# Edward-Sun/DIFUSCO

Hardware: NVIDIA H100
Metric: TSP-500 graphs/sec, 50-step categorical denoise (higher is better)
Workload: dtype f32 (3-term bf16 split on wgmma, fp32 accumulate)

## Files before the change

difusco_b200/csrc/edge_layer_tc.cuh:

```cuda
#pragma once
#include <cuda.h>
#include <cuda_bf16.h>
#include <cuda_runtime.h>

#include <stdlib.h>

#include <string>

#include "common.cuh"
#include "edge_layer_fp32.cuh"

namespace dfb {

constexpr int WG_ROWS = 64;
constexpr int TC_KBLK = 64;
constexpr int TC_KCH = 32;
constexpr int TC_B_BYTES = 256 * TC_KCH * 2;
static_assert(TC_KCH * 2 == 64, "weight chunk rows are one 64-byte swizzle row (tensor map, wgmma_desc_sw64)");
constexpr int TC_A_CHUNK = WG_ROWS * 128;
constexpr int TC_A_BYTES = 8 * TC_A_CHUNK;
constexpr int CONV_BATCH = 16;

constexpr int W_LO_ROWS = H;
constexpr int W_MAT_ROWS = 2 * W_LO_ROWS;
constexpr int W_LAYER_ROWS = 6 * W_MAT_ROWS;
__host__ __device__ constexpr int w_row_C(int l) { return l * W_LAYER_ROWS; }
__host__ __device__ constexpr int w_row_O(int l) { return w_row_C(l) + W_MAT_ROWS; }
__host__ __device__ constexpr int w_row_UVAB(int l) { return w_row_C(l) + 2 * W_MAT_ROWS; }
__host__ __device__ constexpr int w_row_embed(int L, int which) { return L * W_LAYER_ROWS + which * W_MAT_ROWS; }
__host__ __device__ constexpr int w_arena_rows(int L) { return w_row_embed(L, 2); }

template <int NWG>
struct TcCfg {
  static_assert(NWG == 1 || NWG == 2, "one or two consumer warpgroups");
  static constexpr int TILE = NWG * WG_ROWS;
  static constexpr int THREADS = (NWG + 1) * 128;
  static constexpr int NSTAGE = 2 * TC_KBLK / TC_KCH;
  static constexpr int OFF_B = NWG * TC_A_BYTES;
  static constexpr int OFF_PRM = OFF_B + NSTAGE * TC_B_BYTES;
  static constexpr int OFF_ROW = OFF_PRM + 6 * H * 4;
  static constexpr int OFF_SRC = OFF_ROW + TILE * 4;
  static constexpr int OFF_BAR = OFF_SRC + TILE * 8;
  static constexpr int SMEM_BYTES = OFF_BAR + 2 * NSTAGE * 8;
  static constexpr int SMEM_ALLOC = SMEM_BYTES + 1024;
  static constexpr int OFF_TAU = SMEM_BYTES;
  static constexpr int SMEM_ALLOC_TROWS = SMEM_ALLOC + TILE * 8;
  static_assert(SMEM_ALLOC_TROWS <= 232448, "shared memory budget (227 KB per block)");
};

struct TcParams {
  float* e;
  const float* uvab;
  float* partials;
  GraphDev g;
  LayerParams lp;
  const float* tvec;
  const float* xt_lut;
  const float* lut;
  const float* zero_row;
  float* debug_acc;
  const float* lin_in;
  float* lin_out;
  const float* lin_bias;
  int lin_rows;
  int lin_nb;
  int lin_w_row;
  int* error_flag;
  unsigned long long* phase_cycles;
  int write_e, e_zero, agg_mode;
  int w_row_base;
  int n_tiles;
  TimeRows trows;
};

__device__ __forceinline__ uint32_t smem_u32(const void* p) { return (uint32_t)__cvta_generic_to_shared(p); }

__device__ __forceinline__ void mbar_init(uint64_t* bar, uint32_t count) {
  asm volatile("mbarrier.init.shared::cta.b64 [%0], %1;" ::"r"(smem_u32(bar)), "r"(count) : "memory");
}
__device__ __forceinline__ void mbar_arrive(uint64_t* bar) {
  asm volatile("mbarrier.arrive.shared::cta.b64 _, [%0];" ::"r"(smem_u32(bar)) : "memory");
}
__device__ __forceinline__ void mbar_arrive_expect_tx(uint64_t* bar, uint32_t bytes) {
  asm volatile("mbarrier.arrive.expect_tx.shared::cta.b64 _, [%0], %1;" ::"r"(smem_u32(bar)), "r"(bytes) : "memory");
}
__device__ __forceinline__ void mbar_wait(uint64_t* bar, uint32_t parity, int* error_flag, int code) {
  const uint32_t addr = smem_u32(bar);
  uint32_t ok = 0;
#pragma unroll 1
  for (uint32_t spin = 0;; ++spin) {
    asm volatile(
        "{\n .reg .pred p;\n mbarrier.try_wait.parity.shared::cta.b64 p, [%1], %2, %3;\n selp.u32 %0, 1, 0, p;\n}"
        : "=r"(ok)
        : "r"(addr), "r"(parity), "r"(20000u)
        : "memory");
    if (ok) return;
    if (spin > 400000u) {
      if (error_flag) {
        error_flag[1] = (int)blockIdx.x;
        error_flag[2] = (int)parity;
        error_flag[3] = (int)threadIdx.x;
        atomicExch(error_flag, code);
      }
      __threadfence_system();
      __trap();
    }
  }
}
__device__ __forceinline__ void tma_load_2d(uint32_t dst, const CUtensorMap* map, uint64_t* bar, int c0, int c1) {
  asm volatile(
      "cp.async.bulk.tensor.2d.shared::cluster.global.mbarrier::complete_tx::bytes [%0], [%1, {%3, %4}], [%2];"
      ::"r"(dst), "l"(reinterpret_cast<uint64_t>(map)), "r"(smem_u32(bar)), "r"(c0), "r"(c1)
      : "memory");
}
__device__ __forceinline__ void fence_proxy_async() { asm volatile("fence.proxy.async.shared::cta;" ::: "memory"); }
__device__ __forceinline__ void cp_async16(void* dst, const void* src) {
  asm volatile("cp.async.cg.shared.global [%0], [%1], 16;" ::"r"(smem_u32(dst)), "l"(src) : "memory");
}
__device__ __forceinline__ void cp_async_commit() { asm volatile("cp.async.commit_group;" ::: "memory"); }
__device__ __forceinline__ void cp_async_wait_all() { asm volatile("cp.async.wait_group 0;" ::: "memory"); }

__device__ __forceinline__ uint64_t wgmma_desc_sw128(uint32_t smem_addr) {
  return (uint64_t)((smem_addr >> 4) & 0x3fffu) | (1ull << 16) | (64ull << 32) | (1ull << 62);
}
__device__ __forceinline__ uint64_t wgmma_desc_sw64(uint32_t smem_addr) {
  return (uint64_t)((smem_addr >> 4) & 0x3fffu) | (1ull << 16) | (32ull << 32) | (2ull << 62);
}
__device__ __forceinline__ void wgmma_fence() { asm volatile("wgmma.fence.sync.aligned;" ::: "memory"); }
__device__ __forceinline__ void wgmma_commit() { asm volatile("wgmma.commit_group.sync.aligned;" ::: "memory"); }
template <int N>
__device__ __forceinline__ void wgmma_wait() { asm volatile("wgmma.wait_group.sync.aligned %0;" ::"n"(N) : "memory"); }
__device__ __forceinline__ void acc_fence(float (&d)[128]) {
#pragma unroll
  for (int i = 0; i < 128; ++i) asm volatile("" : "+f"(d[i])::"memory");
}
__device__ __forceinline__ void wgmma_bf16(float (&d)[128], uint64_t da, uint64_t db, uint32_t scale_d) {
  asm volatile(
      "{\n .reg .pred p;\n setp.ne.b32 p, %130, 0;\n"
      "wgmma.mma_async.sync.aligned.m64n256k16.f32.bf16.bf16 "
      "{%0, %1, %2, %3, %4, %5, %6, %7, %8, %9, %10, %11, %12, %13, %14, %15, "
      "%16, %17, %18, %19, %20, %21, %22, %23, %24, %25, %26, %27, %28, %29, %30, %31, "
      "%32, %33, %34, %35, %36, %37, %38, %39, %40, %41, %42, %43, %44, %45, %46, %47, "
      "%48, %49, %50, %51, %52, %53, %54, %55, %56, %57, %58, %59, %60, %61, %62, %63, "
      "%64, %65, %66, %67, %68, %69, %70, %71, %72, %73, %74, %75, %76, %77, %78, %79, "
      "%80, %81, %82, %83, %84, %85, %86, %87, %88, %89, %90, %91, %92, %93, %94, %95, "
      "%96, %97, %98, %99, %100, %101, %102, %103, %104, %105, %106, %107, %108, %109, %110, %111, "
      "%112, %113, %114, %115, %116, %117, %118, %119, %120, %121, %122, %123, %124, %125, %126, %127}, "
      "%128, %129, p, 1, 1, 0, 0;\n}"
      : "+f"(d[0]), "+f"(d[1]), "+f"(d[2]), "+f"(d[3]), "+f"(d[4]), "+f"(d[5]), "+f"(d[6]), "+f"(d[7]),
        "+f"(d[8]), "+f"(d[9]), "+f"(d[10]), "+f"(d[11]), "+f"(d[12]), "+f"(d[13]), "+f"(d[14]), "+f"(d[15]),
        "+f"(d[16]), "+f"(d[17]), "+f"(d[18]), "+f"(d[19]), "+f"(d[20]), "+f"(d[21]), "+f"(d[22]), "+f"(d[23]),
        "+f"(d[24]), "+f"(d[25]), "+f"(d[26]), "+f"(d[27]), "+f"(d[28]), "+f"(d[29]), "+f"(d[30]), "+f"(d[31]),
        "+f"(d[32]), "+f"(d[33]), "+f"(d[34]), "+f"(d[35]), "+f"(d[36]), "+f"(d[37]), "+f"(d[38]), "+f"(d[39]),
        "+f"(d[40]), "+f"(d[41]), "+f"(d[42]), "+f"(d[43]), "+f"(d[44]), "+f"(d[45]), "+f"(d[46]), "+f"(d[47]),
        "+f"(d[48]), "+f"(d[49]), "+f"(d[50]), "+f"(d[51]), "+f"(d[52]), "+f"(d[53]), "+f"(d[54]), "+f"(d[55]),
        "+f"(d[56]), "+f"(d[57]), "+f"(d[58]), "+f"(d[59]), "+f"(d[60]), "+f"(d[61]), "+f"(d[62]), "+f"(d[63]),
        "+f"(d[64]), "+f"(d[65]), "+f"(d[66]), "+f"(d[67]), "+f"(d[68]), "+f"(d[69]), "+f"(d[70]), "+f"(d[71]),
        "+f"(d[72]), "+f"(d[73]), "+f"(d[74]), "+f"(d[75]), "+f"(d[76]), "+f"(d[77]), "+f"(d[78]), "+f"(d[79]),
        "+f"(d[80]), "+f"(d[81]), "+f"(d[82]), "+f"(d[83]), "+f"(d[84]), "+f"(d[85]), "+f"(d[86]), "+f"(d[87]),
        "+f"(d[88]), "+f"(d[89]), "+f"(d[90]), "+f"(d[91]), "+f"(d[92]), "+f"(d[93]), "+f"(d[94]), "+f"(d[95]),
        "+f"(d[96]), "+f"(d[97]), "+f"(d[98]), "+f"(d[99]), "+f"(d[100]), "+f"(d[101]), "+f"(d[102]), "+f"(d[103]),
        "+f"(d[104]), "+f"(d[105]), "+f"(d[106]), "+f"(d[107]), "+f"(d[108]), "+f"(d[109]), "+f"(d[110]), "+f"(d[111]),
        "+f"(d[112]), "+f"(d[113]), "+f"(d[114]), "+f"(d[115]), "+f"(d[116]), "+f"(d[117]), "+f"(d[118]), "+f"(d[119]),
        "+f"(d[120]), "+f"(d[121]), "+f"(d[122]), "+f"(d[123]), "+f"(d[124]), "+f"(d[125]), "+f"(d[126]), "+f"(d[127])
      : "l"(da), "l"(db), "r"(scale_d));
}

__device__ __forceinline__ float sigmoid_mufu(float x) {
  float t, r;
  asm("ex2.approx.ftz.f32 %0, %1;" : "=f"(t) : "f"(-1.4426950408889634f * x));
  asm("rcp.approx.ftz.f32 %0, %1;" : "=f"(r) : "f"(1.0f + t));
  return r;
}
__device__ __forceinline__ void split4(float4 x, uint2& hi, uint2& lo) {
  __nv_bfloat162 h01 = __floats2bfloat162_rn(x.x, x.y), h23 = __floats2bfloat162_rn(x.z, x.w);
  float2 f01 = __bfloat1622float2(h01), f23 = __bfloat1622float2(h23);
  __nv_bfloat162 l01 = __floats2bfloat162_rn(x.x - f01.x, x.y - f01.y);
  __nv_bfloat162 l23 = __floats2bfloat162_rn(x.z - f23.x, x.w - f23.y);
  hi.x = *reinterpret_cast<uint32_t*>(&h01);
  hi.y = *reinterpret_cast<uint32_t*>(&h23);
  lo.x = *reinterpret_cast<uint32_t*>(&l01);
  lo.y = *reinterpret_cast<uint32_t*>(&l23);
}
__device__ __forceinline__ void split2(float a, float b, uint32_t& hi, uint32_t& lo) {
  __nv_bfloat162 h = __floats2bfloat162_rn(a, b);
  const float2 f = __bfloat1622float2(h);
  __nv_bfloat162 l = __floats2bfloat162_rn(a - f.x, b - f.y);
  hi = *reinterpret_cast<uint32_t*>(&h);
  lo = *reinterpret_cast<uint32_t*>(&l);
}
__device__ __forceinline__ uint32_t sw128_off(int r, int j) {
  return (uint32_t)((r >> 3) * 1024 + (r & 7) * 128 + ((j ^ (r & 7)) << 4));
}
__device__ __forceinline__ int msg_col(int j, int r) { return 64 * (j >> 3) + ((8 * (j & 7)) ^ (8 * (r & 7))); }
__device__ __forceinline__ float quad_sum(float v) {
  v += __shfl_xor_sync(0xffffffffu, v, 1);
  return v + __shfl_xor_sync(0xffffffffu, v, 2);
}
__device__ __forceinline__ void swap_row_halves(float (&d)[128]) {
#pragma unroll
  for (int j = 0; j < 32; ++j) {
    const float x0 = d[4 * j], x1 = d[4 * j + 1];
    d[4 * j] = d[4 * j + 2];
    d[4 * j + 1] = d[4 * j + 3];
    d[4 * j + 2] = x0;
    d[4 * j + 3] = x1;
  }
}

enum {
  PH_TILES = 0,
  PH_TOTAL,
  PH_CONVERT,
  PH_G1_WAIT,
  PH_G1_MMA,
  PH_E1,
  PH_REDUCE,
  PH_LN,
  PH_G2_WAIT,
  PH_G2_MMA,
  PH_E4,
  PH_COUNT
};

template <int NWG, bool LIN, bool TIMED = false, bool TROWS = false>
__device__ __forceinline__ void edge_layer_wg_body(const CUtensorMap& wmap, const TcParams& P) {
  using Cfg = TcCfg<NWG>;
  constexpr int NSTAGE = Cfg::NSTAGE;
  extern __shared__ unsigned char smem_raw[];
  unsigned char* smem = smem_raw + ((1024u - (smem_u32(smem_raw) & 1023u)) & 1023u);
  float* prm = reinterpret_cast<float*>(smem + Cfg::OFF_PRM);
  int* s_row = reinterpret_cast<int*>(smem + Cfg::OFF_ROW);
  const float** s_src = reinterpret_cast<const float**>(smem + Cfg::OFF_SRC);
  const float** s_tau = reinterpret_cast<const float**>(smem + Cfg::OFF_TAU);
  uint64_t* full = reinterpret_cast<uint64_t*>(smem + Cfg::OFF_BAR);
  uint64_t* empty = full + NSTAGE;

  const int warp = threadIdx.x >> 5, lane = threadIdx.x & 31;
  constexpr bool lin = LIN;
  const int loads_per_tile = (P.write_e ? 2 : 1) * NWG * 4 * NSTAGE;

  if (threadIdx.x == 0) {
    for (int s = 0; s < NSTAGE; ++s) {
      mbar_init(&full[s], 1);
      mbar_init(&empty[s], 4);
    }
    asm volatile("fence.mbarrier_init.release.cluster;" ::: "memory");
    fence_proxy_async();
  }
  for (int i = threadIdx.x; i < H; i += Cfg::THREADS) {
    prm[i] = P.lp.ln_e_g[i];
    prm[H + i] = P.lp.ln_e_b[i];
    prm[2 * H + i] = P.tvec ? P.tvec[i] : 0.0f;
    prm[3 * H + i] = P.lp.ln_o_g[i];
    prm[4 * H + i] = P.lp.ln_o_b[i];
    prm[5 * H + i] = P.lp.b_O[i];
  }
  __syncthreads();
  const uint32_t smem_base = smem_u32(smem);

  if (warp >= 4 * NWG) {
    if constexpr (NWG == 2) asm volatile("setmaxnreg.dec.sync.aligned.u32 40;" ::: "memory");
    if (warp == 4 * NWG && lane == 0) {
      uint32_t u = 0;
      for (int tile = blockIdx.x; tile < P.n_tiles; tile += gridDim.x) {
        for (int i = 0; i < loads_per_tile; ++i, ++u) {
          const int s = u % NSTAGE;
          mbar_wait(&empty[s], ((u / NSTAGE) & 1) ^ 1, P.error_flag, 1);
          mbar_arrive_expect_tx(&full[s], TC_B_BYTES);
          const int row = (lin ? P.lin_w_row + (P.lin_nb == 4 ? (tile & 3) : 0) * W_MAT_ROWS
                               : P.w_row_base + (i >= 4 * NSTAGE * NWG ? w_row_O(0) - w_row_C(0) : 0)) +
                          (s >= NSTAGE / 2 ? W_LO_ROWS : 0);
          const int k = ((i / NSTAGE) & 3) * TC_KBLK + (s % (NSTAGE / 2)) * TC_KCH;
          tma_load_2d(smem_base + Cfg::OFF_B + s * TC_B_BYTES, &wmap, &full[s], k, row);
        }
      }
    }
    return;
  }

  if constexpr (NWG == 2) asm volatile("setmaxnreg.inc.sync.aligned.u32 232;" ::: "memory");
  const int wg = warp >> 2, wi = warp & 3, tid = threadIdx.x & 127;
  const int t4 = lane & 3;
  const int lr0 = wi * 16 + (lane >> 2);
  unsigned char* a_reg = smem + wg * TC_A_BYTES;
  const uint32_t a_base = smem_base + wg * TC_A_BYTES;
  float* msg = reinterpret_cast<float*>(a_reg);
  int* w_row = s_row + wg * WG_ROWS;
  const float** w_src = s_src + wg * WG_ROWS;
  const float** w_tau = s_tau + wg * WG_ROWS;
  auto wg_bar = [&] { asm volatile("bar.sync %0, 128;" ::"r"(1 + wg) : "memory"); };
  const int n_rows = lin ? P.lin_rows : P.g.E;
  float acc[128];

  auto turn_wait = [&] {
    if constexpr (NWG == 2) asm volatile("bar.sync %0, 256;" ::"r"(3 + wg) : "memory");
  };
  auto turn_pass = [&] {
    if constexpr (NWG == 2) asm volatile("bar.arrive %0, 256;" ::"r"(4 - wg) : "memory");
  };
  if (wg == 1) turn_pass();

  uint32_t t_mark = 0, t_start = 0;
  if constexpr (TIMED) t_start = t_mark = (uint32_t)clock();
  auto record = [&](int slot, uint32_t v) {
    if constexpr (TIMED) {
      if (tid == 0) atomicAdd(P.phase_cycles + slot, (unsigned long long)v);
    }
  };
  auto mark = [&](int slot) {
    if constexpr (TIMED) {
      const uint32_t now = (uint32_t)clock();
      record(slot, now - t_mark);
      t_mark = now;
    }
  };

  auto gemm = [&](int wait_slot, int mma_slot) {
    uint32_t waited = 0;
    turn_wait();
    if constexpr (TIMED) t_mark = (uint32_t)clock();
    acc_fence(acc);
    wgmma_fence();
#pragma unroll 1
    for (int kc = 0; kc < 4; ++kc) {
      const uint32_t ahi = a_base + kc * 2 * TC_A_CHUNK, alo = ahi + TC_A_CHUNK;
#pragma unroll
      for (int s = 0; s < NSTAGE; ++s) {
        uint32_t w0 = 0;
        if constexpr (TIMED) w0 = (uint32_t)clock();
        mbar_wait(&full[s], kc & 1, P.error_flag, 2);
        if constexpr (TIMED) waited += (uint32_t)clock() - w0;
        const uint32_t b = smem_base + Cfg::OFF_B + s * TC_B_BYTES;
        const bool b_hi = s < NSTAGE / 2;
#pragma unroll
        for (int k = 0; k < TC_KCH / 16; ++k) {
          const int ks = (s % (NSTAGE / 2)) * (TC_KCH / 16) + k;
          const uint64_t db = wgmma_desc_sw64(b + k * 32);
          wgmma_bf16(acc, wgmma_desc_sw128(ahi + ks * 32), db, (b_hi && ks == 0) ? (uint32_t)(kc != 0) : 1u);
          if (b_hi) wgmma_bf16(acc, wgmma_desc_sw128(alo + ks * 32), db, 1u);
        }
        wgmma_commit();
        wgmma_wait<1>();
        __syncwarp();
        if (lane == 0 && (s > 0 || kc > 0)) mbar_arrive(&empty[(s + NSTAGE - 1) % NSTAGE]);
      }
    }
    wgmma_wait<0>();
    acc_fence(acc);
    __syncwarp();
    if (lane == 0) mbar_arrive(&empty[NSTAGE - 1]);
    turn_pass();
    if constexpr (TIMED) {
      const uint32_t now = (uint32_t)clock();
      record(wait_slot, waited);
      record(mma_slot, now - t_mark - waited);
      t_mark = now;
    }
  };

  auto stage_rows = [&](auto row_src) {
#pragma unroll 1
    for (int i = 0; i < 16; ++i) {
      const int r = wi * 16 + i;
      const float* src = row_src(i) + 4 * lane;
      float* dst = msg + r * H + ((4 * lane) ^ (8 * (r & 7)));
      cp_async16(dst, src);
      cp_async16(dst + 128, src + 128);
    }
    cp_async_commit();
  };

  for (int tile = blockIdx.x; tile < P.n_tiles; tile += gridDim.x) {
    record(PH_TILES, 1);
    const int row_tile = (lin && P.lin_nb == 4) ? (tile >> 2) : tile;
    const int s_base = row_tile * Cfg::TILE + wg * WG_ROWS;
    if (tid < WG_ROWS) {
      const int s = s_base + tid;
      const float* src = P.zero_row;
      int rw = -1;
      if (s < n_rows && lin) {
        src = P.lin_in + (size_t)s * H;
      } else if (s < n_rows) {
        rw = P.g.row[s];
        if (P.e_zero) src = P.zero_row;
        else if (P.xt_lut) src = P.lut + ((P.xt_lut[P.g.perm ? P.g.perm[s] : s] != 0.0f) ? H : 0);
        else src = P.e + (size_t)s * H;
      }
      w_row[tid] = rw;
      w_src[tid] = src;
      if constexpr (TROWS) w_tau[tid] = s < n_rows ? time_row(P.tvec, P.trows, P.g.perm ? P.g.perm[s] : s) : P.zero_row;
    }
    wg_bar();

#pragma unroll 1
    for (int it0 = 0; it0 < 32; it0 += CONV_BATCH) {
      float4 x[CONV_BATCH];
#pragma unroll
      for (int q = 0; q < CONV_BATCH; ++q) {
        const int item = (it0 + q) * 128 + tid;
        x[q] = __ldcg(reinterpret_cast<const float4*>(w_src[item >> 6]) + (item & 63));
      }
#pragma unroll
      for (int q = 0; q < CONV_BATCH; ++q) {
        const int item = (it0 + q) * 128 + tid;
        const int rr = item >> 6, k4 = item & 63;
        uint2 hi, lo;
        split4(x[q], hi, lo);
        const uint32_t off = (k4 >> 4) * 2 * TC_A_CHUNK + sw128_off(rr, (k4 & 15) >> 1) + (k4 & 1) * 8;
        *reinterpret_cast<uint2*>(a_reg + off) = hi;
        *reinterpret_cast<uint2*>(a_reg + off + TC_A_CHUNK) = lo;
      }
    }
    fence_proxy_async();
    wg_bar();
    mark(PH_CONVERT);
    gemm(PH_G1_WAIT, PH_G1_MMA);

    const int sa = s_base + lr0, sb = sa + 8;
    const bool va = sa < n_rows, vb = sb < n_rows;
    if (lin || P.debug_acc) {
      const int nb = (lin && P.lin_nb == 4) ? (tile & 3) : 0;
      const int ostride = lin ? P.lin_nb * H : H;
      float* out = lin ? P.lin_out + nb * H : P.debug_acc;
#pragma unroll
      for (int h = 0; h < 2; ++h) {
        const int s = h ? sb : sa;
        if (!(h ? vb : va)) continue;
#pragma unroll
        for (int j = 0; j < 32; ++j) {
          const int c = 8 * j + 2 * t4;
          float2 o = make_float2(acc[4 * j + 2 * h], acc[4 * j + 2 * h + 1]);
          if (lin) {
            const float2 bb = __ldg(reinterpret_cast<const float2*>(P.lin_bias + nb * H + c));
            o.x += bb.x;
            o.y += bb.y;
          }
          __stcg(reinterpret_cast<float2*>(out + (size_t)s * ostride + c), o);
        }
      }
      continue;
    }

    const int s_lane = s_base + wi * 16 + (lane & 15);
    const int col_lane = s_lane < n_rows ? P.g.col[s_lane] : 0;
    stage_rows([&](int i) { return P.uvab + (size_t)__shfl_sync(0xffffffffu, col_lane, i) * 4 * H + H; });
#pragma unroll 1
    for (int h = 0; h < 2; ++h) {
      const bool v = h ? vb : va;
      const float* ap = P.uvab + (size_t)__shfl_sync(0xffffffffu, col_lane, (lane >> 2) + 8 * h) * 4 * H + 2 * H;
      const float* bp = P.uvab + (size_t)(v ? P.g.row[h ? sb : sa] : 0) * 4 * H + 3 * H;
#pragma unroll
      for (int j = 0; j < 32; ++j) {
        const int c = 8 * j + 2 * t4;
        const float2 ah = __ldg(reinterpret_cast<const float2*>(ap + c));
        const float2 bh = __ldg(reinterpret_cast<const float2*>(bp + c));
        acc[4 * j] = (acc[4 * j] + ah.x) + bh.x;
        acc[4 * j + 1] = (acc[4 * j + 1] + ah.y) + bh.y;
      }
      if (h == 0) {
        cp_async_wait_all();
        __syncwarp();
      }
      float* m = msg + (lr0 + 8 * h) * H + 2 * t4;
#pragma unroll
      for (int j = 0; j < 32; ++j) {
        float2* mp = reinterpret_cast<float2*>(m + msg_col(j, lr0));
        const float2 vh = *mp;
        *mp = make_float2(sigmoid_mufu(acc[4 * j]) * vh.x, sigmoid_mufu(acc[4 * j + 1]) * vh.y);
      }
      swap_row_halves(acc);
    }
    wg_bar();
    mark(PH_E1);
    const bool amax = P.agg_mode == AGG_MAX;
    const float run0 = amax ? -INFINITY : 0.0f;
#pragma unroll 1
    for (int g2 = 0; g2 < WG_ROWS / GROUP; ++g2) {
      const int grp = (s_base >> 5) + g2;
      if (grp >= P.g.n_groups) break;
      const int first_node = P.g.grp_first[grp];
      const size_t pair_base = (size_t)P.g.grp_pair[grp];
      const int node = w_row[g2 * GROUP + lane];
      const int nxt = __shfl_down_sync(0xffffffffu, node, 1);
      const uint32_t ends = __ballot_sync(0xffffffffu, node >= 0 && (lane == GROUP - 1 || nxt != node));
#pragma unroll 1
      for (int cc = 0; cc < 2; ++cc) {
        const int c = tid + 128 * cc;
        float run = run0;
#pragma unroll 8
        for (int r = 0; r < GROUP; ++r) {
          const int lr = g2 * GROUP + r;
          const float m = msg[lr * H + (c ^ (8 * (lr & 7)))];
          run = amax ? fmaxf(run, m) : run + m;
          if ((ends >> r) & 1u) {
            P.partials[(pair_base + (size_t)(w_row[lr] - first_node)) * H + c] = run;
            run = run0;
          }
        }
      }
    }
    wg_bar();
    mark(PH_REDUCE);
    if (!P.write_e) continue;

#pragma unroll 1
    for (int h = 0; h < 2; ++h) {
      float sum = 0.f;
#pragma unroll
      for (int j = 0; j < 32; ++j) sum += acc[4 * j] + acc[4 * j + 1];
      float mean = quad_sum(sum) * (1.0f / H);
      float q = 0.f;
#pragma unroll
      for (int j = 0; j < 32; ++j) {
        const float d0 = acc[4 * j] - mean, d1 = acc[4 * j + 1] - mean;
        q = fmaf(d0, d0, fmaf(d1, d1, q));
      }
      float rstd = rsqrtf(quad_sum(q) * (1.0f / H) + LN_EPS);
      sum = 0.f;
      const float* tau = nullptr;
      if constexpr (TROWS) tau = w_tau[lr0 + 8 * h];
#pragma unroll
      for (int j = 0; j < 32; ++j) {
        const int c = 8 * j + 2 * t4;
        const float2 g = *reinterpret_cast<const float2*>(prm + c);
        const float2 b = *reinterpret_cast<const float2*>(prm + H + c);
        float2 t;
        if constexpr (TROWS) t = __ldg(reinterpret_cast<const float2*>(tau + c));
        else t = *reinterpret_cast<const float2*>(prm + 2 * H + c);
        const float y0 = fmaxf(fmaf((acc[4 * j] - mean) * rstd, g.x, b.x), 0.0f) + t.x;
        const float y1 = fmaxf(fmaf((acc[4 * j + 1] - mean) * rstd, g.y, b.y), 0.0f) + t.y;
        acc[4 * j] = y0;
        acc[4 * j + 1] = y1;
        sum += y0 + y1;
      }
      mean = quad_sum(sum) * (1.0f / H);
      q = 0.f;
#pragma unroll
      for (int j = 0; j < 32; ++j) {
        const float d0 = acc[4 * j] - mean, d1 = acc[4 * j + 1] - mean;
        q = fmaf(d0, d0, fmaf(d1, d1, q));
      }
      rstd = rsqrtf(quad_sum(q) * (1.0f / H) + LN_EPS);
      const int r = lr0 + 8 * h;
#pragma unroll
      for (int j = 0; j < 32; ++j) {
        const int c = 8 * j + 2 * t4;
        const float2 g = *reinterpret_cast<const float2*>(prm + 3 * H + c);
        const float2 b = *reinterpret_cast<const float2*>(prm + 4 * H + c);
        const float z0 = fmaf((acc[4 * j] - mean) * rstd, g.x, b.x);
        const float z1 = fmaf((acc[4 * j + 1] - mean) * rstd, g.y, b.y);
        uint32_t hi, lo;
        split2(z0 * sigmoid_mufu(z0), z1 * sigmoid_mufu(z1), hi, lo);
        const uint32_t off = (j >> 3) * 2 * TC_A_CHUNK + sw128_off(r, j & 7) + 4 * t4;
        *reinterpret_cast<uint32_t*>(a_reg + off) = hi;
        *reinterpret_cast<uint32_t*>(a_reg + off + TC_A_CHUNK) = lo;
      }
      swap_row_halves(acc);
    }
    const float* e_src = w_src[wi * 16 + (lane & 15)];
    fence_proxy_async();
    wg_bar();
    mark(PH_LN);
    gemm(PH_G2_WAIT, PH_G2_MMA);

    stage_rows([&](int i) {
      return reinterpret_cast<const float*>(__shfl_sync(0xffffffffu, reinterpret_cast<unsigned long long>(e_src), i));
    });
    cp_async_wait_all();
    __syncwarp();
#pragma unroll
    for (int h = 0; h < 2; ++h) {
      if (!(h ? vb : va)) continue;
      const int r = lr0 + 8 * h;
      const float* er = msg + r * H + 2 * t4;
      float* dst = P.e + (size_t)(h ? sb : sa) * H;
#pragma unroll
      for (int j = 0; j < 32; ++j) {
        const int c = 8 * j + 2 * t4;
        const float2 ein = *reinterpret_cast<const float2*>(er + msg_col(j, r));
        const float2 bo = *reinterpret_cast<const float2*>(prm + 5 * H + c);
        __stcg(reinterpret_cast<float2*>(dst + c),
               make_float2((ein.x + acc[4 * j + 2 * h]) + bo.x, (ein.y + acc[4 * j + 2 * h + 1]) + bo.y));
      }
    }
    mark(PH_E4);
  }
  if constexpr (TIMED) record(PH_TOTAL, (uint32_t)clock() - t_start);
}

__global__ void __launch_bounds__(TcCfg<2>::THREADS, 1)
k_edge_layer_wg2(const __grid_constant__ CUtensorMap wmap, const TcParams P) {
  edge_layer_wg_body<2, false>(wmap, P);
}
__global__ void __launch_bounds__(TcCfg<2>::THREADS, 1)
k_edge_layer_wg2_timed(const __grid_constant__ CUtensorMap wmap, const TcParams P) {
  edge_layer_wg_body<2, false, true>(wmap, P);
}
__global__ void __launch_bounds__(TcCfg<1>::THREADS, 1)
k_edge_layer_wg1(const __grid_constant__ CUtensorMap wmap, const TcParams P) {
  edge_layer_wg_body<1, false>(wmap, P);
}
__global__ void __launch_bounds__(TcCfg<2>::THREADS, 1)
k_edge_layer_wg2_trows(const __grid_constant__ CUtensorMap wmap, const TcParams P) {
  edge_layer_wg_body<2, false, false, true>(wmap, P);
}
__global__ void __launch_bounds__(TcCfg<1>::THREADS, 1)
k_edge_layer_wg1_trows(const __grid_constant__ CUtensorMap wmap, const TcParams P) {
  edge_layer_wg_body<1, false, false, true>(wmap, P);
}
__global__ void __launch_bounds__(TcCfg<2>::THREADS, 1)
k_linear_wg2(const __grid_constant__ CUtensorMap wmap, const TcParams P) {
  edge_layer_wg_body<2, true>(wmap, P);
}

struct TcState {
  std::string err;
  int num_sms = 0;
  CUtensorMap wmap;
  bool bound = false;
  float* zero_row = nullptr;
  int* error_flag = nullptr;
  int* error_host = nullptr;
  unsigned long long* phase_cycles = nullptr;

  TcState() = default;
  TcState(const TcState&) = delete;
  TcState& operator=(const TcState&) = delete;
  ~TcState() {
    if (zero_row) cudaFree(zero_row);
    if (error_host) cudaFreeHost(error_host);
    if (phase_cycles) cudaFree(phase_cycles);
  }
};

typedef CUresult (*PFN_encodeTiled)(CUtensorMap*, CUtensorMapDataType, cuuint32_t, void*, const cuuint64_t*,
                                    const cuuint64_t*, const cuuint32_t*, const cuuint32_t*, CUtensorMapInterleave,
                                    CUtensorMapSwizzle, CUtensorMapL2promotion, CUtensorMapFloatOOBfill);

inline int tc_init(TcState* st, int num_sms) {
  st->num_sms = num_sms;
  cudaError_t e = cudaFuncSetAttribute(k_edge_layer_wg2, cudaFuncAttributeMaxDynamicSharedMemorySize, TcCfg<2>::SMEM_ALLOC);
  if (e == cudaSuccess)
    e = cudaFuncSetAttribute(k_edge_layer_wg2_timed, cudaFuncAttributeMaxDynamicSharedMemorySize, TcCfg<2>::SMEM_ALLOC);
  if (e == cudaSuccess)
    e = cudaFuncSetAttribute(k_edge_layer_wg1, cudaFuncAttributeMaxDynamicSharedMemorySize, TcCfg<1>::SMEM_ALLOC);
  if (e == cudaSuccess)
    e = cudaFuncSetAttribute(k_edge_layer_wg2_trows, cudaFuncAttributeMaxDynamicSharedMemorySize, TcCfg<2>::SMEM_ALLOC_TROWS);
  if (e == cudaSuccess)
    e = cudaFuncSetAttribute(k_edge_layer_wg1_trows, cudaFuncAttributeMaxDynamicSharedMemorySize, TcCfg<1>::SMEM_ALLOC_TROWS);
  if (e == cudaSuccess)
    e = cudaFuncSetAttribute(k_linear_wg2, cudaFuncAttributeMaxDynamicSharedMemorySize, TcCfg<2>::SMEM_ALLOC);
  if (e != cudaSuccess) {
    st->err = std::string("cudaFuncSetAttribute: ") + cudaGetErrorString(e);
    return -2;
  }
  if ((e = cudaMalloc(&st->zero_row, H * sizeof(float))) != cudaSuccess ||
      (e = cudaMemset(st->zero_row, 0, H * sizeof(float))) != cudaSuccess ||
      (e = cudaMalloc(&st->phase_cycles, 32 * sizeof(unsigned long long))) != cudaSuccess ||
      (e = cudaMemset(st->phase_cycles, 0, 32 * sizeof(unsigned long long))) != cudaSuccess ||
      (e = cudaHostAlloc(&st->error_host, 4 * sizeof(int), cudaHostAllocMapped)) != cudaSuccess ||
      (e = cudaHostGetDevicePointer((void**)&st->error_flag, st->error_host, 0)) != cudaSuccess) {
    st->err = std::string("tc_init alloc: ") + cudaGetErrorString(e);
    return -2;
  }
  return 0;
}

inline int tc_bind_weights(TcState* st, const uint16_t* arena, int L) {
  void* fn = nullptr;
  cudaDriverEntryPointQueryResult qres;
  cudaError_t e = cudaGetDriverEntryPoint("cuTensorMapEncodeTiled", &fn, cudaEnableDefault, &qres);
  if (e != cudaSuccess || !fn || qres != cudaDriverEntryPointSuccess) {
    st->err = "cuTensorMapEncodeTiled entry point not available";
    cudaGetLastError();
    return -2;
  }
  cuuint64_t gdim[2] = {(cuuint64_t)H, (cuuint64_t)w_arena_rows(L)};
  cuuint64_t gstride[1] = {(cuuint64_t)H * sizeof(uint16_t)};
  cuuint32_t box[2] = {(cuuint32_t)TC_KCH, 256u};
  cuuint32_t estr[2] = {1u, 1u};
  CUresult r = ((PFN_encodeTiled)fn)(&st->wmap, CU_TENSOR_MAP_DATA_TYPE_BFLOAT16, 2, (void*)arena, gdim,
                                     gstride, box, estr, CU_TENSOR_MAP_INTERLEAVE_NONE, CU_TENSOR_MAP_SWIZZLE_64B,
                                     CU_TENSOR_MAP_L2_PROMOTION_L2_256B, CU_TENSOR_MAP_FLOAT_OOB_FILL_NONE);
  if (r != CUDA_SUCCESS) {
    st->err = "cuTensorMapEncodeTiled failed with CUresult " + std::to_string((int)r);
    return -2;
  }
  st->bound = true;
  return 0;
}

template <int NWG>
inline int tc_launch(TcState* st, void (*kernel)(CUtensorMap, TcParams), TcParams& P, int rows, int nb,
                     cudaStream_t stream, int smem = TcCfg<NWG>::SMEM_ALLOC) {
  if (!st->bound) {
    st->err = "weights not bound";
    return -1;
  }
  P.zero_row = st->zero_row; P.error_flag = st->error_flag; P.phase_cycles = st->phase_cycles;
  P.n_tiles = nb * ((rows + TcCfg<NWG>::TILE - 1) / TcCfg<NWG>::TILE);
  const int grid = P.n_tiles < st->num_sms ? P.n_tiles : st->num_sms;
  kernel<<<grid, TcCfg<NWG>::THREADS, smem, stream>>>(st->wmap, P);
  const cudaError_t err = cudaGetLastError();
  if (err == cudaSuccess) return 0;
  st->err = std::string("launch: ") + cudaGetErrorString(err);
  return -2;
}

inline int tc_launch_edge_layer(TcState* st, int l, float* e, const float* uvab, float* partials, const GraphDev& g,
                                const LayerParams& lp, const float* tvec, const TimeRows& trows, int write_e,
                                int e_zero, const float* xt_lut, const float* lut, int agg_mode, int nwg, bool timed,
                                float* debug_acc, cudaStream_t stream) {
  TcParams P{};
  P.e = e; P.uvab = uvab; P.partials = partials; P.g = g; P.lp = lp; P.tvec = tvec;
  P.xt_lut = xt_lut; P.lut = lut; P.debug_acc = debug_acc;
  P.write_e = debug_acc ? 0 : write_e;
  P.e_zero = e_zero; P.agg_mode = agg_mode;
  P.w_row_base = w_row_C(l);
  if (trows.index && tvec && !debug_acc) {
    P.trows = trows;
    if (nwg == 1) return tc_launch<1>(st, k_edge_layer_wg1_trows, P, g.E, 1, stream, TcCfg<1>::SMEM_ALLOC_TROWS);
    return tc_launch<2>(st, k_edge_layer_wg2_trows, P, g.E, 1, stream, TcCfg<2>::SMEM_ALLOC_TROWS);
  }
  if (nwg == 1) return tc_launch<1>(st, k_edge_layer_wg1, P, g.E, 1, stream);
  return tc_launch<2>(st, timed && !debug_acc ? k_edge_layer_wg2_timed : k_edge_layer_wg2, P, g.E, 1, stream);
}

inline int tc_launch_linear(TcState* st, const float* in, float* out, const float* bias, int rows, int nb, int w_row,
                            cudaStream_t stream) {
  TcParams P{};
  P.lin_in = in; P.lin_out = out; P.lin_bias = bias; P.lin_rows = rows; P.lin_nb = nb; P.lin_w_row = w_row;
  P.lp.ln_e_g = P.lp.ln_e_b = P.lp.ln_o_g = P.lp.ln_o_b = P.lp.b_O = st->zero_row;
  return tc_launch<2>(st, k_linear_wg2, P, rows, nb, stream);
}

}
```

Before: 23.18.

## Multicast weight chunks across 2-CTA clusters and add L2 evict-first hints

Launches the two-warpgroup edge kernels as 2-CTA clusters. Each CTA fetches half of every weight chunk with TMA multicast into both CTAs, and consumers release ring slots on both the local and the peer empty barriers. This halves the weight traffic from L2 per CTA. Separately, last-use edge-row loads and edge output stores now carry an L2 evict_first policy to protect reused data in L2. In exchange the paired CTAs are coupled, which adds cross-CTA waiting, padded dummy tiles and a grid limited by cluster occupancy.

```diff
diff --git a/difusco_b200/csrc/edge_layer_tc.cuh b/difusco_b200/csrc/edge_layer_tc.cuh
--- a/difusco_b200/csrc/edge_layer_tc.cuh
+++ b/difusco_b200/csrc/edge_layer_tc.cuh
@@ -16,7 +16,10 @@
 constexpr int TC_KBLK = 64;
 constexpr int TC_KCH = 32;
 constexpr int TC_B_BYTES = 256 * TC_KCH * 2;
+constexpr int TC_BOX_ROWS = 128;
+constexpr int TC_B_HALF = TC_BOX_ROWS * TC_KCH * 2;
 static_assert(TC_KCH * 2 == 64, "weight chunk rows are one 64-byte swizzle row (tensor map, wgmma_desc_sw64)");
+static_assert(2 * TC_B_HALF == TC_B_BYTES && TC_B_HALF % 512 == 0, "two boxes per chunk, on 64-byte swizzle periods");
 constexpr int TC_A_CHUNK = WG_ROWS * 128;
 constexpr int TC_A_BYTES = 8 * TC_A_CHUNK;
 constexpr int CONV_BATCH = 16;
@@ -113,11 +116,49 @@
       ::"r"(dst), "l"(reinterpret_cast<uint64_t>(map)), "r"(smem_u32(bar)), "r"(c0), "r"(c1)
       : "memory");
 }
+__device__ __forceinline__ void tma_load_2d_multicast(uint32_t dst, const CUtensorMap* map, uint64_t* bar, int c0, int c1,
+                                                      uint16_t cta_mask) {
+  asm volatile(
+      "cp.async.bulk.tensor.2d.shared::cluster.global.mbarrier::complete_tx::bytes.multicast::cluster"
+      " [%0], [%1, {%3, %4}], [%2], %5;"
+      ::"r"(dst), "l"(reinterpret_cast<uint64_t>(map)), "r"(smem_u32(bar)), "r"(c0), "r"(c1), "h"(cta_mask)
+      : "memory");
+}
+__device__ __forceinline__ uint32_t cluster_ctarank() {
+  uint32_t r;
+  asm volatile("mov.u32 %0, %%cluster_ctarank;" : "=r"(r));
+  return r;
+}
+__device__ __forceinline__ uint32_t mapa_shared(const void* p, uint32_t rank) {
+  uint32_t a;
+  asm volatile("mapa.shared::cluster.u32 %0, %1, %2;" : "=r"(a) : "r"(smem_u32(p)), "r"(rank));
+  return a;
+}
+__device__ __forceinline__ void mbar_arrive_cluster(uint32_t cluster_addr) {
+  asm volatile("mbarrier.arrive.shared::cluster.b64 _, [%0];" ::"r"(cluster_addr) : "memory");
+}
+__device__ __forceinline__ void cluster_arrive() { asm volatile("barrier.cluster.arrive.release;" ::: "memory"); }
+__device__ __forceinline__ void cluster_sync() {
+  cluster_arrive();
+  asm volatile("barrier.cluster.wait.acquire;" ::: "memory");
+}
 __device__ __forceinline__ void fence_proxy_async() { asm volatile("fence.proxy.async.shared::cta;" ::: "memory"); }
 __device__ __forceinline__ void cp_async16(void* dst, const void* src) {
   asm volatile("cp.async.cg.shared.global [%0], [%1], 16;" ::"r"(smem_u32(dst)), "l"(src) : "memory");
 }
 __device__ __forceinline__ void cp_async_commit() { asm volatile("cp.async.commit_group;" ::: "memory"); }
+__device__ __forceinline__ uint64_t l2_evict_first_policy() {
+  uint64_t pol;
+  asm volatile("createpolicy.fractional.L2::evict_first.b64 %0, 1.0;" : "=l"(pol));
+  return pol;
+}
+__device__ __forceinline__ void cp_async16_evict_first(void* dst, const void* src, uint64_t pol) {
+  asm volatile("cp.async.cg.shared.global.L2::cache_hint [%0], [%1], 16, %2;" ::"r"(smem_u32(dst)), "l"(src), "l"(pol)
+               : "memory");
+}
+__device__ __forceinline__ void st_cg_evict_first(float2* p, float2 v, uint64_t pol) {
+  asm volatile("st.global.cg.L2::cache_hint.v2.f32 [%0], {%1, %2}, %3;" ::"l"(p), "f"(v.x), "f"(v.y), "l"(pol) : "memory");
+}
 __device__ __forceinline__ void cp_async_wait_all() { asm volatile("cp.async.wait_group 0;" ::: "memory"); }
 
 __device__ __forceinline__ uint64_t wgmma_desc_sw128(uint32_t smem_addr) {
@@ -223,10 +264,11 @@
   PH_COUNT
 };
 
-template <int NWG, bool LIN, bool TIMED = false, bool TROWS = false>
+template <int NWG, bool LIN, bool CLUSTER, bool TIMED = false, bool TROWS = false>
 __device__ __forceinline__ void edge_layer_wg_body(const CUtensorMap& wmap, const TcParams& P) {
   using Cfg = TcCfg<NWG>;
   constexpr int NSTAGE = Cfg::NSTAGE;
+  static_assert(!CLUSTER || (NWG == 2 && !LIN), "the 2-CTA weight ring serves the two-warpgroup edge kernels");
   extern __shared__ unsigned char smem_raw[];
   unsigned char* smem = smem_raw + ((1024u - (smem_u32(smem_raw) & 1023u)) & 1023u);
   float* prm = reinterpret_cast<float*>(smem + Cfg::OFF_PRM);
@@ -239,11 +281,13 @@
   const int warp = threadIdx.x >> 5, lane = threadIdx.x & 31;
   constexpr bool lin = LIN;
   const int loads_per_tile = (P.write_e ? 2 : 1) * NWG * 4 * NSTAGE;
+  const int n_loop = CLUSTER ? (P.n_tiles + 1) & ~1 : P.n_tiles;
+  const uint32_t rank = CLUSTER ? cluster_ctarank() : 0;
 
   if (threadIdx.x == 0) {
     for (int s = 0; s < NSTAGE; ++s) {
       mbar_init(&full[s], 1);
-      mbar_init(&empty[s], 4);
+      mbar_init(&empty[s], CLUSTER ? 8 : 4);
     }
     asm volatile("fence.mbarrier_init.release.cluster;" ::: "memory");
     fence_proxy_async();
@@ -256,26 +300,34 @@
     prm[4 * H + i] = P.lp.ln_o_b[i];
     prm[5 * H + i] = P.lp.b_O[i];
   }
-  __syncthreads();
+  if constexpr (CLUSTER) cluster_sync();
+  else __syncthreads();
   const uint32_t smem_base = smem_u32(smem);
 
   if (warp >= 4 * NWG) {
     if constexpr (NWG == 2) asm volatile("setmaxnreg.dec.sync.aligned.u32 40;" ::: "memory");
     if (warp == 4 * NWG && lane == 0) {
       uint32_t u = 0;
-      for (int tile = blockIdx.x; tile < P.n_tiles; tile += gridDim.x) {
+      for (int tile = blockIdx.x; tile < n_loop; tile += gridDim.x) {
         for (int i = 0; i < loads_per_tile; ++i, ++u) {
           const int s = u % NSTAGE;
-          mbar_wait(&empty[s], ((u / NSTAGE) & 1) ^ 1, P.error_flag, 1);
+          mbar_wait(&empty[s], ((u / NSTAGE) & 1) ^ 1, P.error_flag, CLUSTER ? 3 : 1);
           mbar_arrive_expect_tx(&full[s], TC_B_BYTES);
           const int row = (lin ? P.lin_w_row + (P.lin_nb == 4 ? (tile & 3) : 0) * W_MAT_ROWS
                                : P.w_row_base + (i >= 4 * NSTAGE * NWG ? w_row_O(0) - w_row_C(0) : 0)) +
                           (s >= NSTAGE / 2 ? W_LO_ROWS : 0);
           const int k = ((i / NSTAGE) & 3) * TC_KBLK + (s % (NSTAGE / 2)) * TC_KCH;
-          tma_load_2d(smem_base + Cfg::OFF_B + s * TC_B_BYTES, &wmap, &full[s], k, row);
+          const uint32_t dst = smem_base + Cfg::OFF_B + s * TC_B_BYTES;
+          if constexpr (CLUSTER) {
+            tma_load_2d_multicast(dst + rank * TC_B_HALF, &wmap, &full[s], k, row + rank * TC_BOX_ROWS, 0b11);
+          } else {
+            tma_load_2d(dst, &wmap, &full[s], k, row);
+            tma_load_2d(dst + TC_B_HALF, &wmap, &full[s], k, row + TC_BOX_ROWS);
+          }
         }
       }
     }
+    if constexpr (CLUSTER) cluster_sync();
     return;
   }
 
@@ -316,7 +368,12 @@
     }
   };
 
-  auto gemm = [&](int wait_slot, int mma_slot) {
+  const uint32_t peer_empty = CLUSTER ? mapa_shared(empty, rank ^ 1u) : 0u;
+  auto release = [&](int s) {
+    mbar_arrive(&empty[s]);
+    if constexpr (CLUSTER) mbar_arrive_cluster(peer_empty + 8 * s);
+  };
+  auto gemm = [&](int wait_slot, int mma_slot, bool closes) {
     uint32_t waited = 0;
     turn_wait();
     if constexpr (TIMED) t_mark = (uint32_t)clock();
@@ -343,13 +400,14 @@
         wgmma_commit();
         wgmma_wait<1>();
         __syncwarp();
-        if (lane == 0 && (s > 0 || kc > 0)) mbar_arrive(&empty[(s + NSTAGE - 1) % NSTAGE]);
+        if (lane == 0 && (s > 0 || kc > 0)) release((s + NSTAGE - 1) % NSTAGE);
       }
     }
     wgmma_wait<0>();
     acc_fence(acc);
     __syncwarp();
-    if (lane == 0) mbar_arrive(&empty[NSTAGE - 1]);
+    if (lane == 0) release(NSTAGE - 1);
+    if (CLUSTER && closes) cluster_arrive();
     turn_pass();
     if constexpr (TIMED) {
       const uint32_t now = (uint32_t)clock();
@@ -359,20 +417,26 @@
     }
   };
 
-  auto stage_rows = [&](auto row_src) {
+  auto stage_rows = [&](auto row_src, bool last_use) {
+    const uint64_t pol = last_use ? l2_evict_first_policy() : 0;
 #pragma unroll 1
     for (int i = 0; i < 16; ++i) {
       const int r = wi * 16 + i;
       const float* src = row_src(i) + 4 * lane;
       float* dst = msg + r * H + ((4 * lane) ^ (8 * (r & 7)));
-      cp_async16(dst, src);
-      cp_async16(dst + 128, src + 128);
+      if (last_use) {
+        cp_async16_evict_first(dst, src, pol);
+        cp_async16_evict_first(dst + 128, src + 128, pol);
+      } else {
+        cp_async16(dst, src);
+        cp_async16(dst + 128, src + 128);
+      }
     }
     cp_async_commit();
   };
 
-  for (int tile = blockIdx.x; tile < P.n_tiles; tile += gridDim.x) {
-    record(PH_TILES, 1);
+  for (int tile = blockIdx.x; tile < n_loop; tile += gridDim.x) {
+    if (tile < P.n_tiles) record(PH_TILES, 1);
     const int row_tile = (lin && P.lin_nb == 4) ? (tile >> 2) : tile;
     const int s_base = row_tile * Cfg::TILE + wg * WG_ROWS;
     if (tid < WG_ROWS) {
@@ -415,7 +479,7 @@
     fence_proxy_async();
     wg_bar();
     mark(PH_CONVERT);
-    gemm(PH_G1_WAIT, PH_G1_MMA);
+    gemm(PH_G1_WAIT, PH_G1_MMA, !P.write_e && tile + (int)gridDim.x >= n_loop);
 
     const int sa = s_base + lr0, sb = sa + 8;
     const bool va = sa < n_rows, vb = sb < n_rows;
@@ -444,7 +508,7 @@
 
     const int s_lane = s_base + wi * 16 + (lane & 15);
     const int col_lane = s_lane < n_rows ? P.g.col[s_lane] : 0;
-    stage_rows([&](int i) { return P.uvab + (size_t)__shfl_sync(0xffffffffu, col_lane, i) * 4 * H + H; });
+    stage_rows([&](int i) { return P.uvab + (size_t)__shfl_sync(0xffffffffu, col_lane, i) * 4 * H + H; }, false);
 #pragma unroll 1
     for (int h = 0; h < 2; ++h) {
       const bool v = h ? vb : va;
@@ -562,11 +626,12 @@
     fence_proxy_async();
     wg_bar();
     mark(PH_LN);
-    gemm(PH_G2_WAIT, PH_G2_MMA);
+    gemm(PH_G2_WAIT, PH_G2_MMA, tile + (int)gridDim.x >= n_loop);
 
     stage_rows([&](int i) {
       return reinterpret_cast<const float*>(__shfl_sync(0xffffffffu, reinterpret_cast<unsigned long long>(e_src), i));
-    });
+    }, true);
+    const uint64_t pol = l2_evict_first_policy();
     cp_async_wait_all();
     __syncwarp();
 #pragma unroll
@@ -580,8 +645,8 @@
         const int c = 8 * j + 2 * t4;
         const float2 ein = *reinterpret_cast<const float2*>(er + msg_col(j, r));
         const float2 bo = *reinterpret_cast<const float2*>(prm + 5 * H + c);
-        __stcg(reinterpret_cast<float2*>(dst + c),
-               make_float2((ein.x + acc[4 * j + 2 * h]) + bo.x, (ein.y + acc[4 * j + 2 * h + 1]) + bo.y));
+        st_cg_evict_first(reinterpret_cast<float2*>(dst + c),
+                          make_float2((ein.x + acc[4 * j + 2 * h]) + bo.x, (ein.y + acc[4 * j + 2 * h + 1]) + bo.y), pol);
       }
     }
     mark(PH_E4);
@@ -589,34 +654,35 @@
   if constexpr (TIMED) record(PH_TOTAL, (uint32_t)clock() - t_start);
 }
 
-__global__ void __launch_bounds__(TcCfg<2>::THREADS, 1)
+__global__ void __cluster_dims__(2, 1, 1) __launch_bounds__(TcCfg<2>::THREADS, 1)
 k_edge_layer_wg2(const __grid_constant__ CUtensorMap wmap, const TcParams P) {
-  edge_layer_wg_body<2, false>(wmap, P);
-}
-__global__ void __launch_bounds__(TcCfg<2>::THREADS, 1)
+  edge_layer_wg_body<2, false, true>(wmap, P);
+}
+__global__ void __cluster_dims__(2, 1, 1) __launch_bounds__(TcCfg<2>::THREADS, 1)
 k_edge_layer_wg2_timed(const __grid_constant__ CUtensorMap wmap, const TcParams P) {
-  edge_layer_wg_body<2, false, true>(wmap, P);
+  edge_layer_wg_body<2, false, true, true>(wmap, P);
 }
 __global__ void __launch_bounds__(TcCfg<1>::THREADS, 1)
 k_edge_layer_wg1(const __grid_constant__ CUtensorMap wmap, const TcParams P) {
-  edge_layer_wg_body<1, false>(wmap, P);
-}
-__global__ void __launch_bounds__(TcCfg<2>::THREADS, 1)
+  edge_layer_wg_body<1, false, false>(wmap, P);
+}
+__global__ void __cluster_dims__(2, 1, 1) __launch_bounds__(TcCfg<2>::THREADS, 1)
 k_edge_layer_wg2_trows(const __grid_constant__ CUtensorMap wmap, const TcParams P) {
-  edge_layer_wg_body<2, false, false, true>(wmap, P);
+  edge_layer_wg_body<2, false, true, false, true>(wmap, P);
 }
 __global__ void __launch_bounds__(TcCfg<1>::THREADS, 1)
 k_edge_layer_wg1_trows(const __grid_constant__ CUtensorMap wmap, const TcParams P) {
-  edge_layer_wg_body<1, false, false, true>(wmap, P);
+  edge_layer_wg_body<1, false, false, false, true>(wmap, P);
 }
 __global__ void __launch_bounds__(TcCfg<2>::THREADS, 1)
 k_linear_wg2(const __grid_constant__ CUtensorMap wmap, const TcParams P) {
-  edge_layer_wg_body<2, true>(wmap, P);
+  edge_layer_wg_body<2, true, false>(wmap, P);
 }
 
 struct TcState {
   std::string err;
   int num_sms = 0;
+  int max_clusters = 0;
   CUtensorMap wmap;
   bool bound = false;
   float* zero_row = nullptr;
@@ -655,6 +721,26 @@
     st->err = std::string("cudaFuncSetAttribute: ") + cudaGetErrorString(e);
     return -2;
   }
+  const struct { const void* fn; int smem; } wg2[] = {{(const void*)k_edge_layer_wg2, TcCfg<2>::SMEM_ALLOC},
+                                                      {(const void*)k_edge_layer_wg2_timed, TcCfg<2>::SMEM_ALLOC},
+                                                      {(const void*)k_edge_layer_wg2_trows, TcCfg<2>::SMEM_ALLOC_TROWS}};
+  st->max_clusters = num_sms / 2;
+  for (const auto& k : wg2) {
+    cudaLaunchConfig_t cfg = {};
+    cfg.gridDim = dim3(2 * (num_sms / 2), 1, 1);
+    cfg.blockDim = dim3(TcCfg<2>::THREADS, 1, 1);
+    cfg.dynamicSmemBytes = k.smem;
+    int n = 0;
+    if ((e = cudaOccupancyMaxActiveClusters(&n, k.fn, &cfg)) != cudaSuccess) {
+      st->err = std::string("cudaOccupancyMaxActiveClusters: ") + cudaGetErrorString(e);
+      return -2;
+    }
+    if (n < st->max_clusters) st->max_clusters = n;
+  }
+  if (st->max_clusters <= 0) {
+    st->err = "no 2-CTA cluster of the edge kernel fits on this device";
+    return -2;
+  }
   if ((e = cudaMalloc(&st->zero_row, H * sizeof(float))) != cudaSuccess ||
       (e = cudaMemset(st->zero_row, 0, H * sizeof(float))) != cudaSuccess ||
       (e = cudaMalloc(&st->phase_cycles, 32 * sizeof(unsigned long long))) != cudaSuccess ||
@@ -678,7 +764,7 @@
   }
   cuuint64_t gdim[2] = {(cuuint64_t)H, (cuuint64_t)w_arena_rows(L)};
   cuuint64_t gstride[1] = {(cuuint64_t)H * sizeof(uint16_t)};
-  cuuint32_t box[2] = {(cuuint32_t)TC_KCH, 256u};
+  cuuint32_t box[2] = {(cuuint32_t)TC_KCH, (cuuint32_t)TC_BOX_ROWS};
   cuuint32_t estr[2] = {1u, 1u};
   CUresult r = ((PFN_encodeTiled)fn)(&st->wmap, CU_TENSOR_MAP_DATA_TYPE_BFLOAT16, 2, (void*)arena, gdim,
                                      gstride, box, estr, CU_TENSOR_MAP_INTERLEAVE_NONE, CU_TENSOR_MAP_SWIZZLE_64B,
@@ -691,7 +777,7 @@
   return 0;
 }
 
-template <int NWG>
+template <int NWG, bool CLUSTER = false>
 inline int tc_launch(TcState* st, void (*kernel)(CUtensorMap, TcParams), TcParams& P, int rows, int nb,
                      cudaStream_t stream, int smem = TcCfg<NWG>::SMEM_ALLOC) {
   if (!st->bound) {
@@ -700,7 +786,9 @@
   }
   P.zero_row = st->zero_row; P.error_flag = st->error_flag; P.phase_cycles = st->phase_cycles;
   P.n_tiles = nb * ((rows + TcCfg<NWG>::TILE - 1) / TcCfg<NWG>::TILE);
-  const int grid = P.n_tiles < st->num_sms ? P.n_tiles : st->num_sms;
+  const int cap = CLUSTER ? 2 * st->max_clusters : st->num_sms;
+  const int want = CLUSTER ? 2 * ((P.n_tiles + 1) / 2) : P.n_tiles;
+  const int grid = want < cap ? want : cap;
   kernel<<<grid, TcCfg<NWG>::THREADS, smem, stream>>>(st->wmap, P);
   const cudaError_t err = cudaGetLastError();
   if (err == cudaSuccess) return 0;
@@ -721,10 +809,10 @@
   if (trows.index && tvec && !debug_acc) {
     P.trows = trows;
     if (nwg == 1) return tc_launch<1>(st, k_edge_layer_wg1_trows, P, g.E, 1, stream, TcCfg<1>::SMEM_ALLOC_TROWS);
-    return tc_launch<2>(st, k_edge_layer_wg2_trows, P, g.E, 1, stream, TcCfg<2>::SMEM_ALLOC_TROWS);
+    return tc_launch<2, true>(st, k_edge_layer_wg2_trows, P, g.E, 1, stream, TcCfg<2>::SMEM_ALLOC_TROWS);
   }
   if (nwg == 1) return tc_launch<1>(st, k_edge_layer_wg1, P, g.E, 1, stream);
-  return tc_launch<2>(st, timed && !debug_acc ? k_edge_layer_wg2_timed : k_edge_layer_wg2, P, g.E, 1, stream);
+  return tc_launch<2, true>(st, timed && !debug_acc ? k_edge_layer_wg2_timed : k_edge_layer_wg2, P, g.E, 1, stream);
 }
 
 inline int tc_launch_linear(TcState* st, const float* in, float* out, const float* bias, int rows, int nb, int w_row,
```

Result: faster. 23.56, median of 6 (+1.6%).
